# NeymarL/ChineseChess-AlphaZero

Measured on NVIDIA H100. Metric: mcts_sims_per_sec, higher is better.
Workload: dtype f16

## Files before the change

chinesechess-alphazero_b200/csrc/cz_igemm.cuh:

```cuda
#pragma once
#include <cuda_fp16.h>
#include "cz_wgmma.cuh"

namespace igemm {

constexpr int kBlockK = 64;
constexpr int kTileM = 128;
constexpr int kAStageBytes = kTileM * 128;
constexpr int kThreads = 384;
constexpr int kConsumerWarps = 8;
constexpr int kSmemLimit = 232448;
constexpr int kMaxStages = 8;

struct Args {
  int n_taps;
  int k_chunks;
  int m_tiles;
  int n_tiles;
  int box_w;
  int box_r;
  int rows;
  int n_total;
  int n_valid;
  int ldo;
  int conv;
  int relu;
  int out_f32;
  const float* bias;
  const __half* residual;
  const float* residual32;
  float* out32;
  void* out;
  uint32_t a_bytes;
  const int* n_dev;
  int rows_per_unit;
  float2* row_stats;
};

__device__ __forceinline__ int args_rows(const Args& a) { return a.n_dev ? __ldg(a.n_dev) * a.rows_per_unit : a.rows; }

template <int N_TILE>
struct Cfg {
  static constexpr int kBStageBytes = N_TILE * 128;
  static constexpr int kStageBytes = kAStageBytes + kBStageBytes;
  static constexpr int kFit = (kSmemLimit - 256 - 1024) / kStageBytes;
  static constexpr int kStages = kFit > kMaxStages ? kMaxStages : kFit;
  static constexpr int kSmemBytes = kStages * kStageBytes + 256 + 1024;
  static_assert(N_TILE % 64 == 0 && N_TILE <= 256, "wgmma N tile");
};

template <int N_TILE>
__global__ void __launch_bounds__(kThreads, 1)
k_igemm(const __grid_constant__ CUtensorMap tmA, const __grid_constant__ CUtensorMap tmB, const Args a) {
  using C = Cfg<N_TILE>;
  constexpr int S = C::kStages;
  extern __shared__ uint8_t smem_raw[];
  uint8_t* smem = reinterpret_cast<uint8_t*>((reinterpret_cast<uintptr_t>(smem_raw) + 1023) & ~(uintptr_t)1023);
  uint64_t* full = reinterpret_cast<uint64_t*>(smem + S * C::kStageBytes);
  uint64_t* empty = full + S;

  const int wgi = threadIdx.x >> 7, t = threadIdx.x & 127;
  if (threadIdx.x == 0) {
    for (int s = 0; s < S; ++s) { wg::mbar_init(&full[s], 1); wg::mbar_init(&empty[s], kConsumerWarps); }
    wg::fence_barrier_init();
  }
  wg::griddep_launch_dependents();
  __syncthreads();
  wg::griddep_wait();

  const int n_kb = a.n_taps * a.k_chunks;
  const int rows = args_rows(a);
  const int m_tiles = a.conv == 1 ? a.m_tiles : (rows + kTileM - 1) / kTileM;
  const int total_tiles = m_tiles * a.n_tiles;

  if (wgi == 0) {
    if (t == 0) {
      wg::prefetch_tmap(&tmA);
      wg::prefetch_tmap(&tmB);
      const uint8_t* skip = a.conv != 2 ? nullptr : a.residual32 ? reinterpret_cast<const uint8_t*>(a.residual32)
                                                                 : reinterpret_cast<const uint8_t*>(a.residual);
      const int skip_es = a.residual32 ? 4 : 2;
      uint32_t s = 0, ph = 0;
      for (int tile = blockIdx.x; tile < total_tiles; tile += gridDim.x) {
        const int m_tile = tile % m_tiles, n_tile = tile / m_tiles;
        const int pix0 = m_tile * kTileM, img0 = pix0 / 90, row0 = (pix0 % 90) / 9, col0 = pix0 % 9;
        for (int tap = 0; tap < a.n_taps; ++tap) {
          const int dy = a.n_taps == 9 ? tap / 3 - 1 : 0;
          const int dx = a.n_taps == 9 ? tap % 3 - 1 : 0;
          for (int kc = 0; kc < a.k_chunks; ++kc) {
            if (skip && tap * a.k_chunks + kc == n_kb / 2) {
              const int nr = min(kTileM, rows - pix0);
              const uint8_t* p0 = skip + ((long long)pix0 * a.ldo + n_tile * N_TILE) * skip_es;
              if (N_TILE == a.ldo)
                wg::prefetch_l2_bulk(p0, (uint32_t)(nr * N_TILE * skip_es));
              else
                for (int r = 0; r < nr; ++r) wg::prefetch_l2_bulk(p0 + (long long)r * a.ldo * skip_es, N_TILE * skip_es);
            }
            wg::mbar_wait(&empty[s], ph ^ 1);
            uint8_t* sA = smem + s * C::kStageBytes;
            uint8_t* sB = sA + kAStageBytes;
            wg::mbar_expect_tx(&full[s], a.a_bytes + (uint32_t)C::kBStageBytes);
            if (a.conv == 2)
              wg::tma_load_im2col_4d(sA, &tmA, &full[s], kc * kBlockK, col0 - 1, row0 - 1, img0, (uint16_t)(dx + 1), (uint16_t)(dy + 1));
            else
              wg::tma_load_3d(sA, &tmA, &full[s], kc * kBlockK, dx, m_tile * a.box_r + dy);
            wg::tma_load_2d(sB, &tmB, &full[s], kc * kBlockK, tap * a.n_total + n_tile * N_TILE);
            if (++s == (uint32_t)S) { s = 0; ph ^= 1; }
          }
        }
      }
    }
    return;
  }

  const int cw = wgi - 1, warp = t >> 5, lane = t & 31;
  const int mrow = cw * 64 + warp * 16 + (lane >> 2);
  const int cq = 2 * (lane & 3);
  float acc[N_TILE / 2];
  uint32_t s = 0, ph = 0;
  for (int tile = blockIdx.x; tile < total_tiles; tile += gridDim.x) {
    const int m_tile = tile % m_tiles, n_tile = tile / m_tiles;
    uint32_t prev = 0;
    for (int kb = 0; kb < n_kb; ++kb) {
      wg::mbar_wait(&full[s], ph);
      const uint32_t sA = wg::smem_u32(smem + s * C::kStageBytes);
      const uint64_t da = wg::smem_desc_sw128(sA + cw * 64 * 128);
      const uint64_t db = wg::smem_desc_sw128(sA + kAStageBytes);
      wg::wgmma_fence();
#pragma unroll
      for (int k = 0; k < kBlockK / 16; ++k)
        wg::Wgmma<N_TILE>::mma(acc, da + (uint64_t)(k * 2), db + (uint64_t)(k * 2), (kb | k) != 0);
      wg::wgmma_commit();
      wg::wgmma_wait<1>();
      if (kb > 0 && lane == 0) wg::mbar_arrive(&empty[prev]);
      prev = s;
      if (++s == (uint32_t)S) { s = 0; ph ^= 1; }
    }
    wg::wgmma_wait<0>();
    if (lane == 0) wg::mbar_arrive(&empty[prev]);

    const int nb = n_tile * N_TILE + cq;
    if (a.bias) {
#pragma unroll
      for (int j = 0; j < N_TILE / 8; ++j) {
        const float2 b = __ldg(reinterpret_cast<const float2*>(a.bias + nb + 8 * j));
        acc[4 * j] += b.x; acc[4 * j + 1] += b.y; acc[4 * j + 2] += b.x; acc[4 * j + 3] += b.y;
      }
    }
    auto out_row = [&](int h, long long& grow, bool& valid, bool& zero) {
      const int m = mrow + 8 * h;
      zero = false;
      if (a.conv == 1) {
        const int srow = m_tile * a.box_r + m / 9;
        valid = m < a.box_r * 9 && srow < rows;
        zero = (srow % 11) == 10;
        grow = (long long)m_tile * a.box_r * 9 + m;
      } else {
        grow = (long long)m_tile * kTileM + m;
        valid = grow < rows;
      }
    };
    if (!a.out_f32 && (a.residual32 || a.residual)) {
#pragma unroll
      for (int h = 0; h < 2; ++h) {
        long long grow;
        bool valid, zero;
        out_row(h, grow, valid, zero);
        if (!valid) continue;
        if (a.residual32) {
          const float* r32 = a.residual32 + grow * a.ldo;
#pragma unroll
          for (int j = 0; j < N_TILE / 8; ++j) {
            const float2 r = __ldg(reinterpret_cast<const float2*>(r32 + nb + 8 * j));
            acc[4 * j + 2 * h] += r.x; acc[4 * j + 2 * h + 1] += r.y;
          }
        } else {
          const __half* r16 = a.residual + grow * a.ldo;
#pragma unroll
          for (int j = 0; j < N_TILE / 8; ++j) {
            const float2 r = __half22float2(__ldg(reinterpret_cast<const __half2*>(r16 + nb + 8 * j)));
            acc[4 * j + 2 * h] += r.x; acc[4 * j + 2 * h + 1] += r.y;
          }
        }
      }
    }
#pragma unroll
    for (int h = 0; h < 2; ++h) {
      long long grow;
      bool valid, zero;
      out_row(h, grow, valid, zero);
      if (a.out_f32) {
        if (a.row_stats) {
          float mx = -INFINITY;
#pragma unroll
          for (int j = 0; j < N_TILE / 8; ++j) {
            if (nb + 8 * j < a.n_valid) mx = fmaxf(mx, acc[4 * j + 2 * h]);
            if (nb + 8 * j + 1 < a.n_valid) mx = fmaxf(mx, acc[4 * j + 2 * h + 1]);
          }
          mx = fmaxf(mx, __shfl_xor_sync(0xffffffffu, mx, 1));
          mx = fmaxf(mx, __shfl_xor_sync(0xffffffffu, mx, 2));
          float sum = 0.f;
#pragma unroll
          for (int j = 0; j < N_TILE / 8; ++j) {
            if (nb + 8 * j < a.n_valid) sum += __expf(acc[4 * j + 2 * h] - mx);
            if (nb + 8 * j + 1 < a.n_valid) sum += __expf(acc[4 * j + 2 * h + 1] - mx);
          }
          sum += __shfl_xor_sync(0xffffffffu, sum, 1);
          sum += __shfl_xor_sync(0xffffffffu, sum, 2);
          if (valid && (lane & 3) == 0) a.row_stats[grow * a.n_tiles + n_tile] = make_float2(mx, sum);
        }
        if (!valid) continue;
        float* o = reinterpret_cast<float*>(a.out) + grow * a.ldo;
#pragma unroll
        for (int j = 0; j < N_TILE / 8; ++j) {
          const int n = nb + 8 * j;
          float x0 = acc[4 * j + 2 * h], x1 = acc[4 * j + 2 * h + 1];
          if (a.relu) { x0 = fmaxf(x0, 0.f); x1 = fmaxf(x1, 0.f); }
          if (n + 1 < a.n_valid) *reinterpret_cast<float2*>(o + n) = make_float2(x0, x1);
          else if (n < a.n_valid) o[n] = x0;
        }
      } else {
        if (!valid) continue;
        __half* o = reinterpret_cast<__half*>(a.out) + grow * a.ldo;
        float* o32 = a.out32 ? a.out32 + grow * a.ldo : nullptr;
#pragma unroll
        for (int j = 0; j < N_TILE / 8; ++j) {
          const int n = nb + 8 * j;
          float x0 = acc[4 * j + 2 * h], x1 = acc[4 * j + 2 * h + 1];
          if (a.relu) { x0 = fmaxf(x0, 0.f); x1 = fmaxf(x1, 0.f); }
          if (zero) { x0 = 0.f; x1 = 0.f; }
          *reinterpret_cast<__half2*>(o + n) = __floats2half2_rn(x0, x1);
          if (o32) *reinterpret_cast<float2*>(o32 + n) = make_float2(x0, x1);
        }
      }
    }
  }
}

}
```

chinesechess-alphazero_b200/csrc/cz_nn.cu:

```cuda
#include <cuda.h>
#include <cuda_fp16.h>
#include <cuda_runtime.h>
#include <math.h>
#include <stdio.h>
#include <stdlib.h>
#include <string.h>
#include <string>
#include <vector>

#include "cz_err.h"
#include "cz_igemm.cuh"
#include "cz_nn.cuh"
#include "cz_nn_host.cuh"

namespace cznn {

#define CZ_CUDA(x)                                                                           \
  do {                                                                                       \
    cudaError_t e__ = (x);                                                                   \
    if (e__ != cudaSuccess) return cz_fail(CZ_ERR_CUDA, "%s: %s", #x, cudaGetErrorString(e__)); \
  } while (0)

constexpr int kLabels = CZ_N_LABELS;
constexpr int kPolN = 2304;
// ... 10 lines not shown

static int load_encode() {
  if (g_encode) return 0;
  void* fn = nullptr;
  cudaDriverEntryPointQueryResult qres;
  cudaError_t e = cudaGetDriverEntryPoint("cuTensorMapEncodeTiled", &fn, cudaEnableDefault, &qres);
  if (e != cudaSuccess || !fn) return cz_fail(CZ_ERR_CUDA, "cuTensorMapEncodeTiled not available: %s", cudaGetErrorString(e));
  g_encode = (EncodeTiledFn)fn;
  fn = nullptr;
  e = cudaGetDriverEntryPoint("cuTensorMapEncodeIm2col", &fn, cudaEnableDefault, &qres);
  if (e == cudaSuccess && fn) g_encode_im2col = (EncodeIm2colFn)fn;
  return 0;
}

int make_map_im2col(CUtensorMap* m, const void* base, int c, long long n_images, int pixels) {
  if (load_encode()) return CZ_ERR_CUDA;
  if (!g_encode_im2col) return cz_fail(CZ_ERR_UNSUPPORTED, "cuTensorMapEncodeIm2col not available");
  cuuint64_t dims[4] = {(cuuint64_t)c, 9, 10, (cuuint64_t)n_images};
  cuuint64_t strides[3] = {(cuuint64_t)c * 2, (cuuint64_t)c * 2 * 9, (cuuint64_t)c * 2 * 90};
  int lower[2] = {-1, -1}, upper[2] = {-1, -1};
  cuuint32_t es[4] = {1, 1, 1, 1};
  CUresult r = g_encode_im2col(m, CU_TENSOR_MAP_DATA_TYPE_FLOAT16, 4, const_cast<void*>(base), dims, strides, lower, upper, 64, (cuuint32_t)pixels,
                               es, CU_TENSOR_MAP_INTERLEAVE_NONE, CU_TENSOR_MAP_SWIZZLE_128B, CU_TENSOR_MAP_L2_PROMOTION_L2_256B,
                               CU_TENSOR_MAP_FLOAT_OOB_FILL_NONE);
  if (r != CUDA_SUCCESS) return cz_fail(CZ_ERR_CUDA, "cuTensorMapEncodeIm2col failed: %d", (int)r);
  return 0;
}

static int make_map_3d(CUtensorMap* m, const void* base, int c, int w, long long rows, int box_w, int box_r) {
  if (load_encode()) return CZ_ERR_CUDA;
  cuuint64_t dims[3] = {(cuuint64_t)c, (cuuint64_t)w, (cuuint64_t)rows};
  cuuint64_t strides[2] = {(cuuint64_t)c * 2, (cuuint64_t)c * 2 * w};
  cuuint32_t box[3] = {64, (cuuint32_t)box_w, (cuuint32_t)box_r};
  cuuint32_t es[3] = {1, 1, 1};
  CUresult r = g_encode(m, CU_TENSOR_MAP_DATA_TYPE_FLOAT16, 3, const_cast<void*>(base), dims, strides, box, es,
                        CU_TENSOR_MAP_INTERLEAVE_NONE, CU_TENSOR_MAP_SWIZZLE_128B, CU_TENSOR_MAP_L2_PROMOTION_L2_256B,
                        CU_TENSOR_MAP_FLOAT_OOB_FILL_NONE);
  if (r != CUDA_SUCCESS) return cz_fail(CZ_ERR_CUDA, "cuTensorMapEncodeTiled(3d) failed: %d", (int)r);
  return 0;
}
int make_map_2d(CUtensorMap* m, const void* base, int k, long long rows, int box_rows) {
  if (load_encode()) return CZ_ERR_CUDA;
  cuuint64_t dims[2] = {(cuuint64_t)k, (cuuint64_t)rows};
  cuuint64_t strides[1] = {(cuuint64_t)k * 2};
  cuuint32_t box[2] = {64, (cuuint32_t)box_rows};
  cuuint32_t es[2] = {1, 1};
  CUresult r = g_encode(m, CU_TENSOR_MAP_DATA_TYPE_FLOAT16, 2, const_cast<void*>(base), dims, strides, box, es,
                        CU_TENSOR_MAP_INTERLEAVE_NONE, CU_TENSOR_MAP_SWIZZLE_128B, CU_TENSOR_MAP_L2_PROMOTION_L2_256B,
                        CU_TENSOR_MAP_FLOAT_OOB_FILL_NONE);
  if (r != CUDA_SUCCESS) return cz_fail(CZ_ERR_CUDA, "cuTensorMapEncodeTiled(2d) failed: %d", (int)r);
  return 0;
}

static int g_num_sms = 0;
int num_sms() {
  if (!g_num_sms) {
    int dev = 0;
    cudaGetDevice(&dev);
    cudaDeviceGetAttribute(&g_num_sms, cudaDevAttrMultiProcessorCount, dev);
    if (g_num_sms <= 0) g_num_sms = 132;
  }
  return g_num_sms;
}

static bool use_pdl() {
  static int pdl = -1;
  if (pdl < 0) { const char* e = getenv("CZ_PDL"); pdl = (e && e[0] == '0') ? 0 : 1; }
  return pdl == 1;
}
template <int N_TILE>
static int launch_igemm_t(const CUtensorMap& tmA, const CUtensorMap& tmB, const igemm::Args& a, cudaStream_t st) {
  using C = igemm::Cfg<N_TILE>;
  static bool attr_set = false;
  if (!attr_set) {
    CZ_CUDA(cudaFuncSetAttribute(igemm::k_igemm<N_TILE>, cudaFuncAttributeMaxDynamicSharedMemorySize, C::kSmemBytes));
    attr_set = true;
  }
  const int tiles = a.m_tiles * a.n_tiles;
  if (tiles <= 0) return 0;
  const int grid = tiles < num_sms() ? tiles : num_sms();
  if (use_pdl()) {
    cudaLaunchConfig_t lc;
    memset(&lc, 0, sizeof(lc));
    lc.gridDim = dim3(grid); lc.blockDim = dim3(igemm::kThreads); lc.dynamicSmemBytes = C::kSmemBytes; lc.stream = st;
    cudaLaunchAttribute at[1];
    at[0].id = cudaLaunchAttributeProgrammaticStreamSerialization;
    at[0].val.programmaticStreamSerializationAllowed = 1;
    lc.attrs = at; lc.numAttrs = 1;
    CZ_CUDA(cudaLaunchKernelEx(&lc, igemm::k_igemm<N_TILE>, tmA, tmB, a));
  } else {
    igemm::k_igemm<N_TILE><<<grid, igemm::kThreads, C::kSmemBytes, st>>>(tmA, tmB, a);
  }
  CZ_CUDA(cudaGetLastError());
  return 0;
}
int launch_igemm(int n_tile, const CUtensorMap& tmA, const CUtensorMap& tmB, const igemm::Args& a, cudaStream_t st) {
  switch (n_tile) {
    case 64: return launch_igemm_t<64>(tmA, tmB, a, st);
    case 128: return launch_igemm_t<128>(tmA, tmB, a, st);
    case 192: return launch_igemm_t<192>(tmA, tmB, a, st);
    case 256: return launch_igemm_t<256>(tmA, tmB, a, st);
  }
  return cz_fail(CZ_ERR_UNSUPPORTED, "igemm: unsupported N tile %d (filters must be 64/128/192/256)", n_tile);
}
static bool use_n_split(int n_boards, int c) {
  static int on = -1;
  if (on < 0) { const char* e = getenv("CZ_NSPLIT"); on = (e && e[0] == '0') ? 0 : 1; }
  if (!on || c <= 64) return false;
  const int m_tiles = (n_boards * 90 + igemm::kTileM - 1) / igemm::kTileM;
  return m_tiles * (c / 64) <= num_sms();
}
static bool use_im2col() {
  static int v = -1;
  if (v < 0) { const char* e = getenv("CZ_CONV_STRIP"); v = (e && e[0] == '1') ? 0 : 1; }
  return v == 1;
}

static igemm::Args conv_args(int n_boards, int c, const float* bias, const __half* residual, __half* out, int relu) {
  igemm::Args a;
  memset(&a, 0, sizeof(a));
  a.n_taps = 9; a.k_chunks = c / 64; a.box_w = 9; a.box_r = 14;
  a.rows = n_boards * 11; a.m_tiles = (a.rows + 13) / 14; a.n_tiles = 1;
  a.n_total = c; a.n_valid = c; a.ldo = c; a.conv = 1; a.relu = relu; a.out_f32 = 0;
  a.bias = bias; a.residual = residual; a.out = out; a.a_bytes = 64 * 9 * 14 * 2;
  return a;
}

static igemm::Args conv_args_dense(int n_boards, int c, const float* bias, const __half* residual, __half* out, int relu) {
  igemm::Args a = conv_args(n_boards, c, bias, residual, out, relu);
  a.conv = 2; a.rows = n_boards * 90; a.m_tiles = (a.rows + 127) / 128; a.a_bytes = 128 * 128;
  return a;
}

static igemm::Args dense_args(int m, int n_valid, int n_pad, int k_pad, int n_tile, const float* bias, float* out, int ldo) {
  igemm::Args a;
  memset(&a, 0, sizeof(a));
  a.n_taps = 1; a.k_chunks = k_pad / 64; a.box_w = 1; a.box_r = 128;
  a.rows = m; a.m_tiles = (m + 127) / 128; a.n_tiles = n_pad / n_tile;
  a.n_total = n_pad; a.n_valid = n_valid; a.ldo = ldo; a.conv = 0; a.relu = 0; a.out_f32 = 1;
  a.bias = bias; a.residual = nullptr; a.out = out; a.a_bytes = 64 * 128 * 2;
  return a;
}

__device__ __forceinline__ int plane_of(uint8_t c) { return c == 0 ? -1 : ((c & 8) ? c - 2 : c - 1); }

__global__ void k_conv_first(const uint8_t* __restrict__ boards, const __half* __restrict__ w,
                             const float* __restrict__ shift, __half* __restrict__ out, float* __restrict__ out32, int c_out,
                             int board_pixels, int in_planes, int board_stride, const int* __restrict__ n_dev) {
  if ((int)blockIdx.x >= __ldg(n_dev)) return;
  __shared__ int8_t pl[2][90];
  __shared__ uint16_t rows[90][52];
  __shared__ uint8_t cnt[90];
  const int b = blockIdx.x, t = threadIdx.x;
  const int n_boards = in_planes / 14;
// ... 237 lines not shown
__global__ void k_copy_pad(const float* src, float* dst, int n_src, int n_dst) {
  const int i = blockIdx.x * blockDim.x + threadIdx.x;
  if (i < n_dst) dst[i] = i < n_src ? src[i] : 0.f;
}

struct Carver {
  uint8_t* base; size_t off, cap;
  void* take(size_t bytes) {
    off = (off + 1023) & ~(size_t)1023;
    void* p = base ? base + off : nullptr;
    off += bytes;
    return p;
  }
};

struct NetWeights {
  __half* w_first; float* shift_first;
  __half* w_conv;  float* shift_conv;
  float *wh, *shifth, *wv1, *bv1, *wv2, *bv2;
  __half* w_pol; float* b_pol;
  CUtensorMap map_wpol;
  std::vector<CUtensorMap> map_w, map_w_64;
  bool ready;
};

struct NnRuntime {
  int filters, blocks, value_fc, max_batch;
  int pol_c, val_c, pol_k1;
  NetWeights nets[2]; int n_nets, cur;
  cudaStream_t stream;
  bool ready;
  uint64_t launches;
  __half *x, *t, *y, *pol_feat;
  float *x32, *y32;
  float* logits;
  float2* stats;
  int* n_scalar;
  bool heads_attr;
  bool capturing;
  size_t prof_open;
  uint8_t* boards_tmp;
  int in_planes;
  __half* w_first; float* shift_first;
  __half* w_conv;  float* shift_conv;
  float *wh, *shifth, *wv1, *bv1, *wv2, *bv2;
  __half* w_pol; float* b_pol;
  float* scratch;
  CUtensorMap map_x, map_t, map_y, map_pf, map_wpol;
  std::vector<CUtensorMap> map_w;
  std::vector<CUtensorMap> map_w_64;
  bool fp32_skip;
  int board_pixels;
  CUtensorMap imap_x, imap_t, imap_y;
  bool profile;
  std::vector<cudaEvent_t> ev;
  size_t ev_used;
  std::vector<double> ev_flops;
  double prof_ms, prof_flops; uint64_t prof_launches;
};

static void store_net(NnRuntime* r, int k) {
  NetWeights& n = r->nets[k];
  n.w_first = r->w_first; n.shift_first = r->shift_first; n.w_conv = r->w_conv; n.shift_conv = r->shift_conv;
  n.wh = r->wh; n.shifth = r->shifth; n.wv1 = r->wv1; n.bv1 = r->bv1; n.wv2 = r->wv2; n.bv2 = r->bv2;
  n.w_pol = r->w_pol; n.b_pol = r->b_pol; n.map_wpol = r->map_wpol; n.map_w = r->map_w; n.map_w_64 = r->map_w_64;
  n.ready = r->ready;
}
static void select_net(NnRuntime* r, int k) {
  if (r->cur == k) return;
  store_net(r, r->cur);
  const NetWeights& n = r->nets[k];
  r->w_first = n.w_first; r->shift_first = n.shift_first; r->w_conv = n.w_conv; r->shift_conv = n.shift_conv;
  r->wh = n.wh; r->shifth = n.shifth; r->wv1 = n.wv1; r->bv1 = n.bv1; r->wv2 = n.wv2; r->bv2 = n.bv2;
  r->w_pol = n.w_pol; r->b_pol = n.b_pol; r->map_wpol = n.map_wpol; r->map_w = n.map_w; r->map_w_64 = n.map_w_64;
  r->ready = n.ready;
  r->cur = k;
}

static void prof_collect(NnRuntime* r) {
  for (size_t i = 0; i + 1 < r->ev_used; i += 2) {
    float ms = 0.f;
    if (cudaEventElapsedTime(&ms, r->ev[i], r->ev[i + 1]) == cudaSuccess) {
      r->prof_ms += ms; r->prof_flops += r->ev_flops[i / 2]; r->prof_launches += (uint64_t)(2 * r->blocks);
    }
  }
  r->ev_used = 0;
}

static void layout(NnRuntime* r, Carver& cv) {
  const int c = r->filters;
  const size_t act = (size_t)r->max_batch * 11 * 9 * c * sizeof(__half);
  r->x = (__half*)cv.take(act);
  r->t = (__half*)cv.take(act);
  r->y = (__half*)cv.take(act);
  r->x32 = (float*)cv.take(act * 2);
  r->y32 = (float*)cv.take(act * 2);
  r->pol_feat = (__half*)cv.take(((size_t)r->max_batch + 128) * 3 * r->pol_k1 * sizeof(__half));
  r->logits = (float*)cv.take((size_t)r->max_batch * kPolN * sizeof(float));
  r->stats = (float2*)cv.take((size_t)r->max_batch * (kPolN / 256) * sizeof(float2));
  r->n_scalar = (int*)cv.take(64);
  r->boards_tmp = (uint8_t*)cv.take((size_t)r->max_batch * 2 * CZ_BOARD_STRIDE);
  for (int net = 0; net < r->n_nets; ++net) {
  r->w_first = (__half*)cv.take((size_t)25 * 28 * c * sizeof(__half));
  r->shift_first = (float*)cv.take(c * sizeof(float));
  r->w_conv = (__half*)cv.take((size_t)2 * r->blocks * 9 * c * c * sizeof(__half));
  r->shift_conv = (float*)cv.take((size_t)2 * r->blocks * c * sizeof(float));
// ... 6 lines not shown
  r->w_pol = (__half*)cv.take((size_t)kPolN * 3 * r->pol_k1 * sizeof(__half));
  r->b_pol = (float*)cv.take(kPolN * sizeof(float));
  r->ready = false;
  r->cur = net;
  store_net(r, net);
  }
  if (r->n_nets > 1) { r->cur = r->n_nets - 1; select_net(r, 0); }
  r->cur = 0;
  r->scratch = (float*)cv.take((size_t)(2 * 256 + 2 * kMaxHeadOut) * sizeof(float));
}

static void set_heads(NnRuntime* r, int pol_c, int val_c) {
  r->pol_c = pol_c > 0 ? pol_c : 4; r->val_c = val_c > 0 ? val_c : 2;
  r->pol_k1 = (r->pol_c * 90 + 63) / 64 * 64;
}
size_t nn_workspace_bytes(int filters, int blocks, int value_fc, int max_batch, int n_nets, int pol_c, int val_c) {
  NnRuntime tmp;
  tmp.filters = filters; tmp.blocks = blocks; tmp.value_fc = value_fc; tmp.max_batch = max_batch; tmp.n_nets = n_nets; tmp.cur = 0;
  set_heads(&tmp, pol_c, val_c);
  Carver cv{nullptr, 0, 0};
  layout(&tmp, cv);
  return cv.off + 4096;
}

NnRuntime* nn_create(int device, int filters, int blocks, int value_fc, int max_batch, void* workspace, size_t bytes,
                     void* stream, int fp32_skip_mode, int n_nets, int in_planes, int pol_c, int val_c) {
  (void)device;
  if (filters % 64 != 0 || filters < 64 || filters > 256) { cz_fail(CZ_ERR_UNSUPPORTED, "nn: filters must be 64..256 step 64"); return nullptr; }
  if (value_fc > 256 || value_fc < 1) { cz_fail(CZ_ERR_UNSUPPORTED, "nn: value_fc_size must be <= 256"); return nullptr; }
  if (n_nets < 1 || n_nets > 2) { cz_fail(CZ_ERR_ARG, "nn: 1 or 2 networks"); return nullptr; }
  if (pol_c < 0 || val_c < 0 || pol_c > 32 || val_c > 4 || (pol_c > 0 ? pol_c : 4) + (val_c > 0 ? val_c : 2) > kMaxHeadOut) {
    cz_fail(CZ_ERR_UNSUPPORTED, "nn: head widths up to 32 policy / 4 value channels"); return nullptr;
  }
  if (bytes < nn_workspace_bytes(filters, blocks, value_fc, max_batch, n_nets, pol_c, val_c)) { cz_fail(CZ_ERR_ARG, "nn: workspace too small"); return nullptr; }
  NnRuntime* r = new NnRuntime();
  set_heads(r, pol_c, val_c);
  r->heads_attr = false;
  r->filters = filters; r->blocks = blocks; r->value_fc = value_fc; r->max_batch = max_batch; r->n_nets = n_nets; r->cur = 0;
  r->stream = (cudaStream_t)stream; r->ready = false; r->launches = 0;
  r->in_planes = in_planes == 28 ? 28 : 14;
  r->fp32_skip = fp32_skip_mode == 1 || (fp32_skip_mode == 0 && blocks >= 10);
  { const char* e = getenv("CZ_FP32_SKIP"); if (e && e[0] == '1') r->fp32_skip = true; if (e && e[0] == '0') r->fp32_skip = false; }
  r->profile = false; r->ev_used = 0; r->prof_ms = 0; r->prof_flops = 0; r->prof_launches = 0; r->capturing = false;
  Carver cv{(uint8_t*)workspace, 0, bytes};
  layout(r, cv);
  const int c = filters;
  const long long rows = (long long)max_batch * 11;
  int rc = 0;
  r->board_pixels = use_im2col() ? 90 : 99;
  if (r->board_pixels == 90) {
    rc |= make_map_im2col(&r->imap_x, r->x, c, max_batch);
    rc |= make_map_im2col(&r->imap_t, r->t, c, max_batch);
    rc |= make_map_im2col(&r->imap_y, r->y, c, max_batch);
  }
  rc |= make_map_3d(&r->map_x, r->x, c, 9, rows, 9, 14);
  rc |= make_map_3d(&r->map_t, r->t, c, 9, rows, 9, 14);
  rc |= make_map_3d(&r->map_y, r->y, c, 9, rows, 9, 14);
  rc |= make_map_3d(&r->map_pf, r->pol_feat, 3 * r->pol_k1, 1, (long long)max_batch + 128, 1, 128);
  for (int net = n_nets - 1; net >= 0; --net) {
    select_net(r, net);
    rc |= make_map_2d(&r->map_wpol, r->w_pol, 3 * r->pol_k1, kPolN, 256);
    r->map_w.resize(2 * blocks);
    r->map_w_64.resize(2 * blocks);
    for (int i = 0; i < 2 * blocks; ++i) {
      rc |= make_map_2d(&r->map_w[i], r->w_conv + (size_t)i * 9 * c * c, c, 9LL * c, c);
      rc |= make_map_2d(&r->map_w_64[i], r->w_conv + (size_t)i * 9 * c * c, c, 9LL * c, 64);
    }
    store_net(r, net);
  }
  if (rc) { delete r; return nullptr; }
  cudaMemsetAsync(r->x, 0, (size_t)max_batch * 11 * 9 * c * 2, r->stream);
  cudaMemsetAsync(r->t, 0, (size_t)max_batch * 11 * 9 * c * 2, r->stream);
  cudaMemsetAsync(r->y, 0, (size_t)max_batch * 11 * 9 * c * 2, r->stream);
  cudaMemsetAsync(r->pol_feat, 0, ((size_t)max_batch + 128) * 3 * r->pol_k1 * 2, r->stream);
  return r;
}

void nn_destroy(NnRuntime* r) {
  if (!r) return;
  for (cudaEvent_t e : r->ev) cudaEventDestroy(e);
  delete r;
}
void nn_profile(NnRuntime* r, bool on) { if (r) { r->profile = on; } }
int nn_profile_read(NnRuntime* r, double* ms, uint64_t* launches, double* flops) {
  if (!r) return cz_fail(CZ_ERR_STATE, "no network");
  CZ_CUDA(cudaStreamSynchronize(r->stream));
  prof_collect(r);
  if (ms) *ms = r->prof_ms;
  if (launches) *launches = r->prof_launches;
  if (flops) *flops = r->prof_flops;
  r->prof_ms = 0; r->prof_flops = 0; r->prof_launches = 0;
  return 0;
}
bool nn_ready(const NnRuntime* r) {
  if (!r) return false;
  for (int k = 0; k < r->n_nets; ++k)
    if (!(k == r->cur ? r->ready : r->nets[k].ready)) return false;
  return true;
}
uint64_t nn_launches(const NnRuntime* r) { return r ? r->launches : 0; }

struct WeightSet {
  const cz_tensor_desc* d; int n;
  const cz_tensor_desc* find(const std::string& layer, const std::string& weight) const {
    for (int i = 0; i < n; ++i) {
      std::string nm = d[i].name ? d[i].name : "";
// ... 78 lines not shown
    CZ_CUDA(cudaMemcpyAsync(r->wv1, k1->dev, (size_t)r->val_c * 90 * h * 4, cudaMemcpyDeviceToDevice, st));
    CZ_CUDA(cudaMemcpyAsync(r->bv1, b1->dev, (size_t)h * 4, cudaMemcpyDeviceToDevice, st));
    CZ_CUDA(cudaMemcpyAsync(r->wv2, k2->dev, (size_t)h * 4, cudaMemcpyDeviceToDevice, st));
    CZ_CUDA(cudaMemcpyAsync(r->bv2, b2->dev, 4, cudaMemcpyDeviceToDevice, st));
  }
  r->launches += 6 + 2 * r->blocks;
  CZ_CUDA(cudaGetLastError());
  CZ_CUDA(cudaStreamSynchronize(st));
  r->ready = true;
  return 0;
}

static int conv_first_threads(int c) {
  const int pairs = c / 2;
  int g = 256 / pairs;
  if (g < 1) g = 1;
  while (pairs * g < 96) ++g;
  return pairs * g;
}
static int fw_first(NnRuntime* r, const uint8_t* boards, int n, const int* n_dev) {
  const int c = r->filters;
  const bool s32 = r->board_pixels == 90 && r->fp32_skip;
  int slices = (2 * num_sms() + n - 1) / n;
  if (slices > 15) slices = 15;
  k_conv_first<<<dim3(n, slices), conv_first_threads(c), 0, r->stream>>>(boards, r->w_first, r->shift_first, r->x, s32 ? r->x32 : nullptr, c, r->board_pixels,
                                                            r->in_planes, (r->in_planes / 14) * CZ_BOARD_STRIDE, n_dev);
  r->launches++;
  CZ_CUDA(cudaGetLastError());
  return 0;
}
static int fw_tower(NnRuntime* r, int n, const int* n_dev) {
  const int c = r->filters;
  cudaStream_t st = r->stream;
  const bool dense = r->board_pixels == 90;
  const bool s32 = dense && r->fp32_skip;
  float *x32 = s32 ? r->x32 : nullptr, *y32 = s32 ? r->y32 : nullptr;
  CUtensorMap *ix = &r->imap_x, *iy = &r->imap_y;
  __half *x = r->x, *y = r->y;
  CUtensorMap *mx = &r->map_x, *my = &r->map_y;
  for (int i = 0; i < r->blocks; ++i) {
    const size_t wsz = (size_t)c;
    igemm::Args a1 = conv_args(n, c, r->shift_conv + (size_t)(2 * i) * wsz, nullptr, r->t, 1);
    igemm::Args a2 = conv_args(n, c, r->shift_conv + (size_t)(2 * i + 1) * wsz, x, y, 1);
    if (dense) {
      igemm::Args d1 = conv_args_dense(n, c, a1.bias, nullptr, r->t, 1);
      igemm::Args d2 = conv_args_dense(n, c, a2.bias, x, y, 1);
      d1.n_dev = n_dev; d1.rows_per_unit = 90; d2.n_dev = n_dev; d2.rows_per_unit = 90;
      d2.residual32 = x32; d2.out32 = y32;
      { float* t32 = x32; x32 = y32; y32 = t32; }
      const bool split = use_n_split(n, c);
      const int nt = split ? 64 : c;
      const std::vector<CUtensorMap>& wm = split ? r->map_w_64 : r->map_w;
      d1.n_tiles = d2.n_tiles = c / nt;
      if (launch_igemm(nt, *ix, wm[2 * i], d1, st)) return CZ_ERR_CUDA;
      if (launch_igemm(nt, r->imap_t, wm[2 * i + 1], d2, st)) return CZ_ERR_CUDA;
      CUtensorMap* ti = ix; ix = iy; iy = ti;
    } else {
      if (launch_igemm(c, *mx, r->map_w[2 * i], a1, st)) return CZ_ERR_CUDA;
      if (launch_igemm(c, r->map_t, r->map_w[2 * i + 1], a2, st)) return CZ_ERR_CUDA;
    }
    r->launches += 2;
    __half* tx = x; x = y; y = tx;
    CUtensorMap* tm = mx; mx = my; my = tm;
  }
  return 0;
}
static int fw_heads(NnRuntime* r, int n, const int* n_dev, float* value) {
  const int c = r->filters;
  const bool s32 = r->board_pixels == 90 && r->fp32_skip;
  const bool odd = (r->blocks & 1) != 0;
  const __half* x = odd ? r->y : r->x;
  const float* x32 = s32 ? (odd ? r->y32 : r->x32) : nullptr;
  const size_t hsm = heads_smem_bytes(c, r->pol_c + r->val_c);
  if (hsm > 48 * 1024 && !r->heads_attr) {
    CZ_CUDA(cudaFuncSetAttribute(k_heads, cudaFuncAttributeMaxDynamicSharedMemorySize, (int)hsm));
    r->heads_attr = true;
  }
  const int hp = n <= 2 * num_sms() ? 1 : kHeadPos;
  k_heads<<<(n + hp - 1) / hp, 256, hsm, r->stream>>>(x, x32, c, n_dev, r->board_pixels, r->pol_c, r->val_c, r->pol_k1, r->wh, r->shifth,
                                                      r->wv1, r->bv1, r->wv2, r->bv2, r->value_fc, r->pol_feat, value, hp);
  igemm::Args ap = dense_args(n, kLabels, kPolN, 3 * r->pol_k1, 256, r->b_pol, r->logits, kPolN);
  ap.n_dev = n_dev; ap.rows_per_unit = 1; ap.row_stats = r->stats;
  if (launch_igemm(256, r->map_pf, r->map_wpol, ap, r->stream)) return CZ_ERR_CUDA;
  r->launches += 2;
  CZ_CUDA(cudaGetLastError());
  return 0;
}
void nn_prof_begin(NnRuntime* r, double flops) {
  r->prof_open = (size_t)-1;
  if (!r->profile) return;
  if (r->ev_used + 2 > 4096) { cudaStreamSynchronize(r->stream); prof_collect(r); }
  while (r->ev.size() < r->ev_used + 2) { cudaEvent_t e; cudaEventCreate(&e); r->ev.push_back(e); }
  r->prof_open = r->ev_used; r->ev_used += 2;
  if (r->ev_flops.size() < r->ev_used / 2) r->ev_flops.resize(r->ev_used / 2);
  r->ev_flops[r->prof_open / 2] = flops > 0 ? flops : 0.0;
  cudaEventRecord(r->ev[r->prof_open], r->stream);
}
void nn_prof_end(NnRuntime* r) {
  if (r->prof_open != (size_t)-1) cudaEventRecord(r->ev[r->prof_open + 1], r->stream);
  r->prof_open = (size_t)-1;
}
static int forward_tower(NnRuntime* r, const uint8_t* boards, int n_max, const int* n_dev, float* value) {
  int rc = fw_first(r, boards, n_max, n_dev);
  if (rc) return rc;
  nn_prof_begin(r, 2.0 * 90.0 * 9.0 * r->filters * r->filters * (double)n_max * 2.0 * r->blocks);
  rc = fw_tower(r, n_max, n_dev);
  nn_prof_end(r);
// ... 143 lines not shown
```

chinesechess-alphazero_b200/csrc/cz_nn_host.cuh:

```cuda
#pragma once
#include <cuda.h>
#include <cuda_runtime.h>

namespace igemm { struct Args; }

namespace cznn {

int make_map_im2col(CUtensorMap* m, const void* base, int c, long long n_images, int pixels = 128);
int make_map_2d(CUtensorMap* m, const void* base, int k, long long rows, int box_rows);
int num_sms();
int launch_igemm(int n_tile, const CUtensorMap& tmA, const CUtensorMap& tmB, const igemm::Args& a, cudaStream_t st);

}
```

chinesechess-alphazero_b200/csrc/cz_wgmma.cuh:

```cuda
#pragma once
#include <cuda.h>
#include <cuda_runtime.h>
#include <stdint.h>

namespace wg {

__device__ __forceinline__ uint32_t smem_u32(const void* p) { return (uint32_t)__cvta_generic_to_shared(p); }

__device__ __forceinline__ void mbar_init(uint64_t* bar, uint32_t count) {
  asm volatile("mbarrier.init.shared::cta.b64 [%0], %1;" ::"r"(smem_u32(bar)), "r"(count) : "memory");
}
__device__ __forceinline__ void fence_barrier_init() { asm volatile("fence.mbarrier_init.release.cluster;" ::: "memory"); }
__device__ __forceinline__ void mbar_expect_tx(uint64_t* bar, uint32_t bytes) {
  asm volatile("mbarrier.arrive.expect_tx.shared::cta.b64 _, [%0], %1;" ::"r"(smem_u32(bar)), "r"(bytes) : "memory");
}
__device__ __forceinline__ void mbar_arrive(uint64_t* bar) {
  asm volatile("mbarrier.arrive.shared::cta.b64 _, [%0];" ::"r"(smem_u32(bar)) : "memory");
}
__device__ __forceinline__ void mbar_wait(uint64_t* bar, uint32_t parity) {
  const uint32_t addr = smem_u32(bar);
  uint32_t ok;
  do {
    asm volatile(
        "{\n\t.reg .pred p;\n\t"
        "mbarrier.try_wait.parity.shared::cta.b64 p, [%1], %2;\n\t"
        "selp.u32 %0, 1, 0, p;\n\t}"
        : "=r"(ok)
        : "r"(addr), "r"(parity)
        : "memory");
  } while (!ok);
}

__device__ __forceinline__ void prefetch_tmap(const CUtensorMap* t) {
  asm volatile("prefetch.tensormap [%0];" ::"l"(reinterpret_cast<uint64_t>(t)) : "memory");
}
__device__ __forceinline__ void tma_load_2d(void* dst, const CUtensorMap* t, uint64_t* bar, int c0, int c1) {
  asm volatile(
      "cp.async.bulk.tensor.2d.shared::cluster.global.mbarrier::complete_tx::bytes [%0], [%1, {%3, %4}], [%2];"
      ::"r"(smem_u32(dst)), "l"(reinterpret_cast<uint64_t>(t)), "r"(smem_u32(bar)), "r"(c0), "r"(c1)
      : "memory");
}
__device__ __forceinline__ void tma_load_3d(void* dst, const CUtensorMap* t, uint64_t* bar, int c0, int c1, int c2) {
  asm volatile(
      "cp.async.bulk.tensor.3d.shared::cluster.global.mbarrier::complete_tx::bytes [%0], [%1, {%3, %4, %5}], [%2];"
      ::"r"(smem_u32(dst)), "l"(reinterpret_cast<uint64_t>(t)), "r"(smem_u32(bar)), "r"(c0), "r"(c1), "r"(c2)
      : "memory");
}
__device__ __forceinline__ void prefetch_l2_bulk(const void* p, uint32_t bytes) {
  asm volatile("cp.async.bulk.prefetch.L2.global [%0], %1;" ::"l"((uint64_t)__cvta_generic_to_global(p)), "r"(bytes) : "memory");
}
__device__ __forceinline__ void tma_load_im2col_4d(void* dst, const CUtensorMap* t, uint64_t* bar, int c, int w, int h, int n,
                                                   uint16_t ow, uint16_t oh) {
  asm volatile(
      "cp.async.bulk.tensor.4d.shared::cluster.global.im2col.mbarrier::complete_tx::bytes [%0], [%1, {%3, %4, %5, %6}], [%2], {%7, %8};"
      ::"r"(smem_u32(dst)), "l"(reinterpret_cast<uint64_t>(t)), "r"(smem_u32(bar)), "r"(c), "r"(w), "r"(h), "r"(n), "h"(ow), "h"(oh)
      : "memory");
}

__device__ __forceinline__ void griddep_launch_dependents() { asm volatile("griddepcontrol.launch_dependents;" ::: "memory"); }
__device__ __forceinline__ void griddep_wait() { asm volatile("griddepcontrol.wait;" ::: "memory"); }

__device__ __forceinline__ uint64_t smem_desc_sw128(uint32_t saddr) {
  uint64_t d = 0;
  d |= (uint64_t)((saddr >> 4) & 0x3FFF);
  d |= (uint64_t)1 << 16;
  d |= (uint64_t)(1024 >> 4) << 32;
  d |= (uint64_t)1 << 62;
  return d;
}
__device__ __forceinline__ void wgmma_fence() { asm volatile("wgmma.fence.sync.aligned;" ::: "memory"); }
__device__ __forceinline__ void wgmma_commit() { asm volatile("wgmma.commit_group.sync.aligned;" ::: "memory"); }
template <int N>
__device__ __forceinline__ void wgmma_wait() { asm volatile("wgmma.wait_group.sync.aligned %0;" ::"n"(N) : "memory"); }

template <int N>
struct Wgmma;
template <>
struct Wgmma<64> {
  __device__ __forceinline__ static void mma(float (&d)[32], uint64_t da, uint64_t db, uint32_t accumulate) {
    asm volatile(
        "{\n\t.reg .pred p;\n\t"
        "setp.ne.b32 p, %34, 0;\n\t"
        "wgmma.mma_async.sync.aligned.m64n64k16.f32.f16.f16 "
        "{%0, %1, %2, %3, %4, %5, %6, %7, %8, %9, %10, %11, %12, %13, %14, %15, %16, %17, %18, %19, %20, %21, %22, %23, %24, %25, %26, %27, %28, %29, %30, %31}, "
        "%32, %33, p, 1, 1, 0, 0;\n\t}"
        : "+f"(d[0]), "+f"(d[1]), "+f"(d[2]), "+f"(d[3]), "+f"(d[4]), "+f"(d[5]), "+f"(d[6]), "+f"(d[7]), "+f"(d[8]), "+f"(d[9]), "+f"(d[10]), "+f"(d[11]), "+f"(d[12]), "+f"(d[13]), "+f"(d[14]), "+f"(d[15]), "+f"(d[16]), "+f"(d[17]), "+f"(d[18]), "+f"(d[19]), "+f"(d[20]), "+f"(d[21]), "+f"(d[22]), "+f"(d[23]), "+f"(d[24]), "+f"(d[25]), "+f"(d[26]), "+f"(d[27]), "+f"(d[28]), "+f"(d[29]), "+f"(d[30]), "+f"(d[31])
        : "l"(da), "l"(db), "r"(accumulate));
  }
};
template <>
struct Wgmma<128> {
  __device__ __forceinline__ static void mma(float (&d)[64], uint64_t da, uint64_t db, uint32_t accumulate) {
    asm volatile(
        "{\n\t.reg .pred p;\n\t"
        "setp.ne.b32 p, %66, 0;\n\t"
        "wgmma.mma_async.sync.aligned.m64n128k16.f32.f16.f16 "
        "{%0, %1, %2, %3, %4, %5, %6, %7, %8, %9, %10, %11, %12, %13, %14, %15, %16, %17, %18, %19, %20, %21, %22, %23, %24, %25, %26, %27, %28, %29, %30, %31, %32, %33, %34, %35, %36, %37, %38, %39, %40, %41, %42, %43, %44, %45, %46, %47, %48, %49, %50, %51, %52, %53, %54, %55, %56, %57, %58, %59, %60, %61, %62, %63}, "
        "%64, %65, p, 1, 1, 0, 0;\n\t}"
        : "+f"(d[0]), "+f"(d[1]), "+f"(d[2]), "+f"(d[3]), "+f"(d[4]), "+f"(d[5]), "+f"(d[6]), "+f"(d[7]), "+f"(d[8]), "+f"(d[9]), "+f"(d[10]), "+f"(d[11]), "+f"(d[12]), "+f"(d[13]), "+f"(d[14]), "+f"(d[15]), "+f"(d[16]), "+f"(d[17]), "+f"(d[18]), "+f"(d[19]), "+f"(d[20]), "+f"(d[21]), "+f"(d[22]), "+f"(d[23]), "+f"(d[24]), "+f"(d[25]), "+f"(d[26]), "+f"(d[27]), "+f"(d[28]), "+f"(d[29]), "+f"(d[30]), "+f"(d[31]), "+f"(d[32]), "+f"(d[33]), "+f"(d[34]), "+f"(d[35]), "+f"(d[36]), "+f"(d[37]), "+f"(d[38]), "+f"(d[39]), "+f"(d[40]), "+f"(d[41]), "+f"(d[42]), "+f"(d[43]), "+f"(d[44]), "+f"(d[45]), "+f"(d[46]), "+f"(d[47]), "+f"(d[48]), "+f"(d[49]), "+f"(d[50]), "+f"(d[51]), "+f"(d[52]), "+f"(d[53]), "+f"(d[54]), "+f"(d[55]), "+f"(d[56]), "+f"(d[57]), "+f"(d[58]), "+f"(d[59]), "+f"(d[60]), "+f"(d[61]), "+f"(d[62]), "+f"(d[63])
        : "l"(da), "l"(db), "r"(accumulate));
// ... 56 lines not shown
```

Before: 123,300.

## Stage igemm epilogue through swizzled shared memory and TMA bulk stores

For the first conv of each residual block (no residual, f16 output, full M tiles), consumer warpgroups write bias+ReLU results into a triple-buffered 64B-swizzled shared ring and issue TMA 2D stores per 32-column slice instead of scattered per-thread global half2 stores. Per-slot mbarriers and bulk read-group waits handle slot reuse, and a new tensor map for the intermediate buffer is created on the host. Producer/consumer register rebalancing via setmaxnreg is also added. The epilogue ring takes shared memory away from the pipeline, which may cut stage count, and adds barrier and fence overhead.

Result: faster. 129,400 (median of 6 runs) (+4.9%).

```diff
diff --git a/chinesechess-alphazero_b200/csrc/cz_igemm.cuh b/chinesechess-alphazero_b200/csrc/cz_igemm.cuh
--- a/chinesechess-alphazero_b200/csrc/cz_igemm.cuh
+++ b/chinesechess-alphazero_b200/csrc/cz_igemm.cuh
@@ -11,6 +11,10 @@
 constexpr int kConsumerWarps = 8;
 constexpr int kSmemLimit = 232448;
 constexpr int kMaxStages = 8;
+constexpr int kEpiCols = 32;
+constexpr int kEpiSlotBytes = 64 * kEpiCols * 2;
+constexpr int kEpiSlots = 3;
+constexpr int kEpiBytes = kEpiSlots * kEpiSlotBytes;
 
 struct Args {
   int n_taps;
@@ -35,6 +39,7 @@
   const int* n_dev;
   int rows_per_unit;
   float2* row_stats;
+  int staged;
 };
 
 __device__ __forceinline__ int args_rows(const Args& a) { return a.n_dev ? __ldg(a.n_dev) * a.rows_per_unit : a.rows; }
@@ -43,25 +48,30 @@
 struct Cfg {
   static constexpr int kBStageBytes = N_TILE * 128;
   static constexpr int kStageBytes = kAStageBytes + kBStageBytes;
-  static constexpr int kFit = (kSmemLimit - 256 - 1024) / kStageBytes;
+  static constexpr int kFit = (kSmemLimit - 2 * kEpiBytes - 256 - 1024) / kStageBytes;
   static constexpr int kStages = kFit > kMaxStages ? kMaxStages : kFit;
-  static constexpr int kSmemBytes = kStages * kStageBytes + 256 + 1024;
+  static constexpr int kSmemBytes = kStages * kStageBytes + 2 * kEpiBytes + 256 + 1024;
   static_assert(N_TILE % 64 == 0 && N_TILE <= 256, "wgmma N tile");
+  static_assert((2 * kStages + 2 * kEpiSlots) * 8 <= 256, "barrier space");
 };
 
 template <int N_TILE>
 __global__ void __launch_bounds__(kThreads, 1)
-k_igemm(const __grid_constant__ CUtensorMap tmA, const __grid_constant__ CUtensorMap tmB, const Args a) {
+k_igemm(const __grid_constant__ CUtensorMap tmA, const __grid_constant__ CUtensorMap tmB, const __grid_constant__ CUtensorMap tmOut,
+        const Args a) {
   using C = Cfg<N_TILE>;
   constexpr int S = C::kStages;
   extern __shared__ uint8_t smem_raw[];
   uint8_t* smem = reinterpret_cast<uint8_t*>((reinterpret_cast<uintptr_t>(smem_raw) + 1023) & ~(uintptr_t)1023);
-  uint64_t* full = reinterpret_cast<uint64_t*>(smem + S * C::kStageBytes);
+  uint8_t* epi = smem + S * C::kStageBytes;
+  uint64_t* full = reinterpret_cast<uint64_t*>(epi + 2 * kEpiBytes);
   uint64_t* empty = full + S;
+  uint64_t* efree = empty + S;
 
   const int wgi = threadIdx.x >> 7, t = threadIdx.x & 127;
   if (threadIdx.x == 0) {
     for (int s = 0; s < S; ++s) { wg::mbar_init(&full[s], 1); wg::mbar_init(&empty[s], kConsumerWarps); }
+    for (int s = 0; s < 2 * kEpiSlots; ++s) wg::mbar_init(&efree[s], 1);
     wg::fence_barrier_init();
   }
   wg::griddep_launch_dependents();
@@ -73,7 +83,11 @@
   const int m_tiles = a.conv == 1 ? a.m_tiles : (rows + kTileM - 1) / kTileM;
   const int total_tiles = m_tiles * a.n_tiles;
 
+  constexpr int kSteps = N_TILE / kEpiCols;
+  auto tile_staged = [&](int tile) { return a.staged && (tile % m_tiles) * kTileM + kTileM <= rows; };
+
   if (wgi == 0) {
+    wg::reg_dealloc<40>();
     if (t == 0) {
       wg::prefetch_tmap(&tmA);
       wg::prefetch_tmap(&tmB);
@@ -113,10 +127,23 @@
     return;
   }
 
+  wg::reg_alloc<232>();
   const int cw = wgi - 1, warp = t >> 5, lane = t & 31;
   const int mrow = cw * 64 + warp * 16 + (lane >> 2);
   const int cq = 2 * (lane & 3);
   float acc[N_TILE / 2];
+  uint8_t* ering = epi + cw * kEpiBytes;
+  uint64_t* fre = efree + cw * kEpiSlots;
+  const uint32_t erow = warp * 16 + (lane >> 2);
+  const uint32_t e_off = erow * 64 + (lane & 3) * 4, e_x = (erow >> 1) & 3;
+  uint32_t e_slot = 0, e_ph = 0;
+  uint32_t e_issued = 0, e_released = 0, e_rel_slot = 0;
+  auto release_to = [&](uint32_t upto) {
+    for (; e_released < upto; ++e_released) {
+      wg::mbar_arrive(&fre[e_rel_slot]);
+      if (++e_rel_slot == kEpiSlots) e_rel_slot = 0;
+    }
+  };
   uint32_t s = 0, ph = 0;
   for (int tile = blockIdx.x; tile < total_tiles; tile += gridDim.x) {
     const int m_tile = tile % m_tiles, n_tile = tile / m_tiles;
@@ -146,6 +173,35 @@
         const float2 b = __ldg(reinterpret_cast<const float2*>(a.bias + nb + 8 * j));
         acc[4 * j] += b.x; acc[4 * j + 1] += b.y; acc[4 * j + 2] += b.x; acc[4 * j + 3] += b.y;
       }
+    }
+    if (tile_staged(tile)) {
+      if (t == 0) { wg::bulk_wait_group_read<0>(); release_to(e_issued); }
+#pragma unroll
+      for (int st = 0; st < kSteps; ++st) {
+        uint8_t* slot = ering + e_slot * kEpiSlotBytes;
+        wg::mbar_wait(&fre[e_slot], e_ph ^ 1);
+#pragma unroll
+        for (int jj = 0; jj < kEpiCols / 8; ++jj) {
+#pragma unroll
+          for (int h = 0; h < 2; ++h) {
+            const int i = 4 * (st * (kEpiCols / 8) + jj) + 2 * h;
+            float x0 = acc[i], x1 = acc[i + 1];
+            if (a.relu) { x0 = fmaxf(x0, 0.f); x1 = fmaxf(x1, 0.f); }
+            *reinterpret_cast<__half2*>(slot + e_off + h * 8 * 64 + ((jj ^ e_x) << 4)) = __floats2half2_rn(x0, x1);
+          }
+        }
+        wg::fence_proxy_async();
+        wg::named_barrier(1 + cw, 128);
+        if (t == 0) {
+          wg::tma_store_2d(&tmOut, slot, n_tile * N_TILE + st * kEpiCols, m_tile * kTileM + cw * 64);
+          wg::bulk_commit();
+          ++e_issued;
+          wg::bulk_wait_group_read<1>();
+          release_to(e_issued - 1);
+        }
+        if (++e_slot == kEpiSlots) { e_slot = 0; e_ph ^= 1; }
+      }
+      continue;
     }
     auto out_row = [&](int h, long long& grow, bool& valid, bool& zero) {
       const int m = mrow + 8 * h;
@@ -235,6 +291,7 @@
       }
     }
   }
+  if (t == 0) wg::bulk_wait_group_all();
 }
 
 }
diff --git a/chinesechess-alphazero_b200/csrc/cz_nn.cu b/chinesechess-alphazero_b200/csrc/cz_nn.cu
--- a/chinesechess-alphazero_b200/csrc/cz_nn.cu
+++ b/chinesechess-alphazero_b200/csrc/cz_nn.cu
@@ -86,6 +86,19 @@
   return 0;
 }
 
+static int make_map_epi(CUtensorMap* m, const void* base, int cols, long long rows) {
+  if (load_encode()) return CZ_ERR_CUDA;
+  cuuint64_t dims[2] = {(cuuint64_t)cols, (cuuint64_t)rows};
+  cuuint64_t strides[1] = {(cuuint64_t)cols * 2};
+  cuuint32_t box[2] = {(cuuint32_t)igemm::kEpiCols, 64};
+  cuuint32_t es[2] = {1, 1};
+  CUresult r = g_encode(m, CU_TENSOR_MAP_DATA_TYPE_FLOAT16, 2, const_cast<void*>(base), dims, strides, box, es,
+                        CU_TENSOR_MAP_INTERLEAVE_NONE, CU_TENSOR_MAP_SWIZZLE_64B, CU_TENSOR_MAP_L2_PROMOTION_L2_128B,
+                        CU_TENSOR_MAP_FLOAT_OOB_FILL_NONE);
+  if (r != CUDA_SUCCESS) return cz_fail(CZ_ERR_CUDA, "cuTensorMapEncodeTiled(epilogue) failed: %d", (int)r);
+  return 0;
+}
+
 static int g_num_sms = 0;
 int num_sms() {
   if (!g_num_sms) {
@@ -103,7 +116,7 @@
   return pdl == 1;
 }
 template <int N_TILE>
-static int launch_igemm_t(const CUtensorMap& tmA, const CUtensorMap& tmB, const igemm::Args& a, cudaStream_t st) {
+static int launch_igemm_t(const CUtensorMap& tmA, const CUtensorMap& tmB, const CUtensorMap& tmOut, const igemm::Args& a, cudaStream_t st) {
   using C = igemm::Cfg<N_TILE>;
   static bool attr_set = false;
   if (!attr_set) {
@@ -121,19 +134,22 @@
     at[0].id = cudaLaunchAttributeProgrammaticStreamSerialization;
     at[0].val.programmaticStreamSerializationAllowed = 1;
     lc.attrs = at; lc.numAttrs = 1;
-    CZ_CUDA(cudaLaunchKernelEx(&lc, igemm::k_igemm<N_TILE>, tmA, tmB, a));
+    CZ_CUDA(cudaLaunchKernelEx(&lc, igemm::k_igemm<N_TILE>, tmA, tmB, tmOut, a));
   } else {
-    igemm::k_igemm<N_TILE><<<grid, igemm::kThreads, C::kSmemBytes, st>>>(tmA, tmB, a);
+    igemm::k_igemm<N_TILE><<<grid, igemm::kThreads, C::kSmemBytes, st>>>(tmA, tmB, tmOut, a);
   }
   CZ_CUDA(cudaGetLastError());
   return 0;
 }
-int launch_igemm(int n_tile, const CUtensorMap& tmA, const CUtensorMap& tmB, const igemm::Args& a, cudaStream_t st) {
+int launch_igemm(int n_tile, const CUtensorMap& tmA, const CUtensorMap& tmB, const igemm::Args& a0, cudaStream_t st, const CUtensorMap* out_map) {
+  igemm::Args a = a0;
+  a.staged = out_map && a.conv == 2 && !a.out_f32 && !a.residual && !a.residual32 && !a.out32;
+  const CUtensorMap& tmOut = a.staged ? *out_map : tmA;
   switch (n_tile) {
-    case 64: return launch_igemm_t<64>(tmA, tmB, a, st);
-    case 128: return launch_igemm_t<128>(tmA, tmB, a, st);
-    case 192: return launch_igemm_t<192>(tmA, tmB, a, st);
-    case 256: return launch_igemm_t<256>(tmA, tmB, a, st);
+    case 64: return launch_igemm_t<64>(tmA, tmB, tmOut, a, st);
+    case 128: return launch_igemm_t<128>(tmA, tmB, tmOut, a, st);
+    case 192: return launch_igemm_t<192>(tmA, tmB, tmOut, a, st);
+    case 256: return launch_igemm_t<256>(tmA, tmB, tmOut, a, st);
   }
   return cz_fail(CZ_ERR_UNSUPPORTED, "igemm: unsupported N tile %d (filters must be 64/128/192/256)", n_tile);
 }
@@ -477,6 +493,7 @@
   bool fp32_skip;
   int board_pixels;
   CUtensorMap imap_x, imap_t, imap_y;
+  CUtensorMap emap_t;
   bool profile;
   std::vector<cudaEvent_t> ev;
   size_t ev_used;
@@ -589,6 +606,7 @@
     rc |= make_map_im2col(&r->imap_x, r->x, c, max_batch);
     rc |= make_map_im2col(&r->imap_t, r->t, c, max_batch);
     rc |= make_map_im2col(&r->imap_y, r->y, c, max_batch);
+    rc |= make_map_epi(&r->emap_t, r->t, c, (long long)max_batch * 90);
   }
   rc |= make_map_3d(&r->map_x, r->x, c, 9, rows, 9, 14);
   rc |= make_map_3d(&r->map_t, r->t, c, 9, rows, 9, 14);
@@ -773,7 +791,7 @@
       const int nt = split ? 64 : c;
       const std::vector<CUtensorMap>& wm = split ? r->map_w_64 : r->map_w;
       d1.n_tiles = d2.n_tiles = c / nt;
-      if (launch_igemm(nt, *ix, wm[2 * i], d1, st)) return CZ_ERR_CUDA;
+      if (launch_igemm(nt, *ix, wm[2 * i], d1, st, &r->emap_t)) return CZ_ERR_CUDA;
       if (launch_igemm(nt, r->imap_t, wm[2 * i + 1], d2, st)) return CZ_ERR_CUDA;
       CUtensorMap* ti = ix; ix = iy; iy = ti;
     } else {
diff --git a/chinesechess-alphazero_b200/csrc/cz_nn_host.cuh b/chinesechess-alphazero_b200/csrc/cz_nn_host.cuh
--- a/chinesechess-alphazero_b200/csrc/cz_nn_host.cuh
+++ b/chinesechess-alphazero_b200/csrc/cz_nn_host.cuh
@@ -9,6 +9,7 @@
 int make_map_im2col(CUtensorMap* m, const void* base, int c, long long n_images, int pixels = 128);
 int make_map_2d(CUtensorMap* m, const void* base, int k, long long rows, int box_rows);
 int num_sms();
-int launch_igemm(int n_tile, const CUtensorMap& tmA, const CUtensorMap& tmB, const igemm::Args& a, cudaStream_t st);
+int launch_igemm(int n_tile, const CUtensorMap& tmA, const CUtensorMap& tmB, const igemm::Args& a, cudaStream_t st,
+                 const CUtensorMap* out_map = nullptr);
 
 }
diff --git a/chinesechess-alphazero_b200/csrc/cz_wgmma.cuh b/chinesechess-alphazero_b200/csrc/cz_wgmma.cuh
--- a/chinesechess-alphazero_b200/csrc/cz_wgmma.cuh
+++ b/chinesechess-alphazero_b200/csrc/cz_wgmma.cuh
@@ -31,6 +31,14 @@
   } while (!ok);
 }
 
+__device__ __forceinline__ void named_barrier(int id, int threads) {
+  asm volatile("bar.sync %0, %1;" ::"r"(id), "r"(threads) : "memory");
+}
+template <int N>
+__device__ __forceinline__ void reg_dealloc() { asm volatile("setmaxnreg.dec.sync.aligned.u32 %0;" ::"n"(N)); }
+template <int N>
+__device__ __forceinline__ void reg_alloc() { asm volatile("setmaxnreg.inc.sync.aligned.u32 %0;" ::"n"(N)); }
+
 __device__ __forceinline__ void prefetch_tmap(const CUtensorMap* t) {
   asm volatile("prefetch.tensormap [%0];" ::"l"(reinterpret_cast<uint64_t>(t)) : "memory");
 }
@@ -46,6 +54,16 @@
       ::"r"(smem_u32(dst)), "l"(reinterpret_cast<uint64_t>(t)), "r"(smem_u32(bar)), "r"(c0), "r"(c1), "r"(c2)
       : "memory");
 }
+__device__ __forceinline__ void tma_store_2d(const CUtensorMap* t, const void* src, int c0, int c1) {
+  asm volatile("cp.async.bulk.tensor.2d.global.shared::cta.bulk_group [%0, {%2, %3}], [%1];"
+               ::"l"(reinterpret_cast<uint64_t>(t)), "r"(smem_u32(src)), "r"(c0), "r"(c1)
+               : "memory");
+}
+__device__ __forceinline__ void bulk_commit() { asm volatile("cp.async.bulk.commit_group;" ::: "memory"); }
+template <int N>
+__device__ __forceinline__ void bulk_wait_group_read() { asm volatile("cp.async.bulk.wait_group.read %0;" ::"n"(N) : "memory"); }
+__device__ __forceinline__ void bulk_wait_group_all() { asm volatile("cp.async.bulk.wait_group 0;" ::: "memory"); }
+__device__ __forceinline__ void fence_proxy_async() { asm volatile("fence.proxy.async.shared::cta;" ::: "memory"); }
 __device__ __forceinline__ void prefetch_l2_bulk(const void* p, uint32_t bytes) {
   asm volatile("cp.async.bulk.prefetch.L2.global [%0], %1;" ::"l"((uint64_t)__cvta_generic_to_global(p)), "r"(bytes) : "memory");
 }
```
